# koadman/libMems

Hardware: AMD Instinct MI355X
Metric: seed-mers/sec sorted+matched (+ MUMs/sec) at 1/2/4/8 MI355X; HBM GB/s vs roofline (higher is better)
Workload: dtype u64; 1 GPU; BASELINE config 3: 8 x 100 Mbp, seed weight 19 (0x7b974ef), MemHash seed stage (sorted+matched); genomes=8, genome_length=100000000, seedmers_total=799999792, seedmers_rank0=799999792, probes_rank0=100459493, parallelism=1 GPU

## Files before the change

libmems_amd/csrc/groups.hip:

```cpp
#include <cstdlib>
#include <type_traits>

#include "match_device.h"
#include "seed_device.h"

namespace mums {

namespace {

constexpr int kGTile = kSegTile;
constexpr int kGRounds = kGTile / kBlock;
constexpr int kSlots = kGTile / 2;
#ifndef MUMS_GROUP_SPLIT
#define MUMS_GROUP_SPLIT 2
#endif
constexpr int kGSplit = MUMS_GROUP_SPLIT;
constexpr int kGSub = kGTile / kGSplit;
constexpr int kGSubRounds = kGSub / kBlock;
constexpr int kSubSlots = kGSub / 2;
static_assert(kGSub % kBlock == 0 && kGSubRounds * (kBlock / 64) <= 64, "probe sub-tile");

__device__ __forceinline__ uint32_t blk_excl_scan(uint32_t v, uint32_t* s_w, uint32_t* total) {
    const int lane = threadIdx.x & 63, wv = threadIdx.x >> 6;
    uint32_t inc = v;
    #pragma unroll
    for (int d = 1; d < 64; d <<= 1) {
        uint32_t t = __shfl_up(inc, d, 64);
        if (lane >= d) inc += t;
    }
    if (lane == 63) s_w[wv] = inc;
    __syncthreads();
    uint32_t pre = 0, tot = 0;
    #pragma unroll
    for (int w = 0; w < kBlock / 64; ++w) {
        const uint32_t x = s_w[w];
        pre += (w < wv) ? x : 0u;
        tot += x;
    }
    __syncthreads();
    *total = tot;
    return pre + inc - v;
}

template <int MG, typename View>
__global__ __launch_bounds__(kBlock) void probe_tile_kernel(View v, const SegTile* __restrict__ tiles, uint64_t N,
                                                            GenomeTable gt, MatchParams mp, int L,
                                                            uint32_t* __restrict__ tile_count,
                                                            uint64_t* __restrict__ slot_info,
                                                            uint32_t* __restrict__ slot_bucket,
                                                            DevCounters* __restrict__ ctr) {
    __shared__ uint16_t heads[kGTile];
    __shared__ uint32_t okb[kGTile];
    __shared__ uint16_t gsz16[kGTile];
    __shared__ uint32_t wcnt[kGRounds][kBlock / 64];
    __shared__ uint32_t s_w[kBlock / 64];
    __shared__ uint32_t s_red[2];
    const int lane = threadIdx.x & 63, wv = threadIdx.x >> 6;
    const SegTile td = tiles[blockIdx.x];
    if (td.count == 0) {
        if (threadIdx.x == 0) {
            tile_count[blockIdx.x] = 0;
            tile_count[gridDim.x + 32 + blockIdx.x] = 0;
        }
        return;
    }
    const uint64_t tile0 = td.start;
    const uint64_t lt = (lane == 0) ? 0ull : (~0ull >> (64 - lane));

    uint32_t hmask = 0;
    #pragma unroll
    for (int r = 0; r < kGRounds; ++r) {
        const uint32_t q = r * kBlock + threadIdx.x;
        const uint64_t i = tile0 + q;
        bool head = false;
        if (q < td.count) head = (i == td.bstart) || (v.gkey(i) != v.gkey(i - 1));
        hmask |= (head ? 1u : 0u) << r;
        const uint64_t bal = __ballot(head);
        if (lane == 0) wcnt[r][wv] = (uint32_t)__popcll(bal);
    }
    __syncthreads();
    if (threadIdx.x == 0) {
        uint32_t acc = 0;
        for (int r = 0; r < kGRounds; ++r)
            for (int w = 0; w < kBlock / 64; ++w) { const uint32_t c = wcnt[r][w]; wcnt[r][w] = acc; acc += c; }
        s_red[0] = acc;
    }
    __syncthreads();
    #pragma unroll
    for (int r = 0; r < kGRounds; ++r) {
        const bool head = (hmask >> r) & 1u;
        const uint64_t bal = __ballot(head);
        if (head) heads[wcnt[r][wv] + (uint32_t)__popcll(bal & lt)] = (uint16_t)(r * kBlock + threadIdx.x);
    }
    __syncthreads();
    const uint32_t H = s_red[0];

    uint32_t nrep = 0;
    const bool fast = mp.repeat_tol == 0 && mp.enum_tol == 1;
    for (uint32_t j = threadIdx.x; j < H; j += kBlock) {
        uint32_t gsz = 0;
        int64_t off = 0;
        bool ok;
        if (fast) {
            ok = probe_offset_fast<MG, View>(v, tile0 + heads[j], td.bend, gt, mp, L, &off, &gsz);
        } else {
            Mhe<MG> P;
            ok = build_probe<MG, View>(v, tile0 + heads[j], td.bend, gt, mp, L, P, &gsz);
            off = P.offset;
        }
        nrep += gsz > (uint32_t)kRepeatLimit;
        okb[j] = ok ? (0x80000000u | bucket_of(off, mp.table_size)) : 0u;
        gsz16[j] = (uint16_t)(gsz > 65535u ? 65535u : gsz);
    }
    if (nrep) atomicAdd(&ctr->repeat_limit, (unsigned long long)nrep);
    __syncthreads();

    uint32_t base = 0;
    const uint64_t sb = (uint64_t)blockIdx.x * kSlots;
    for (uint32_t c = 0; c < H; c += kBlock) {
        const uint32_t j = c + threadIdx.x;
        const uint32_t vv = j < H ? okb[j] : 0u;
        const uint32_t ok = vv >> 31;
        uint32_t tot;
        const uint32_t o = blk_excl_scan(ok, s_w, &tot);
        if (ok) {
            slot_info[sb + base + o] = (tile0 + heads[j]) | ((uint64_t)gsz16[j] << 32);
            slot_bucket[sb + base + o] = vv & 0x7FFFFFFFu;
        }
        base += tot;
    }
    if (threadIdx.x == 0) {
        tile_count[blockIdx.x] = base;
        tile_count[gridDim.x + 32 + blockIdx.x] = H;
    }
}

typedef __attribute__((address_space(3))) const uint64_t lds_u64;

template <int IB>
struct TileRecViewT {
    lds_u64* lds;
    const uint64_t* glob;
    uint64_t t0;
    uint32_t count;
    __device__ __forceinline__ uint64_t raw(uint64_t i) const {
        const uint64_t k = i - t0;
        return k < count ? lds[k] : glob[i];
    }
    __device__ __forceinline__ uint64_t gkey(uint64_t i) const { return raw(i) >> (IB + 1); }
    __device__ __forceinline__ uint32_t par(uint64_t i) const { return (uint32_t)(raw(i) >> IB) & 1u; }
    __device__ __forceinline__ uint64_t gidx(uint64_t i) const { return raw(i) & ((1ull << IB) - 1); }
    __device__ __forceinline__ RecFields get(uint64_t i) const {
        const uint64_t r = raw(i);
        return RecFields{r >> (IB + 1), (uint32_t)(r >> IB) & 1u, r & ((1ull << IB) - 1)};
    }
};

template <int MG, int IB, bool kGl = false, bool kFastOnly = false>
__global__ __launch_bounds__(kBlock) __attribute__((amdgpu_waves_per_eu(kGl ? 6 : 1))) void probe_tile_rec_kernel(const uint64_t* __restrict__ rec,
                                                                const SegTile* __restrict__ tiles, GenomeTable gt,
                                                                MatchParams mp, int L,
                                                                uint32_t* __restrict__ tile_count,
                                                                uint64_t* __restrict__ slot_info,
                                                                uint32_t* __restrict__ slot_bucket,
                                                                DevCounters* __restrict__ ctr,
                                                                double inv_table) {
    constexpr int kGRounds = kGSubRounds;
    __shared__ uint64_t srec[kGSub];
    __shared__ uint16_t heads[kSubSlots];
    __shared__ uint32_t wcnt[kGRounds * (kBlock / 64)];
    __shared__ uint32_t s_w[kBlock / 64];
    __shared__ uint32_t s_red[2];
    __shared__ uint64_t s_prev, s_next;
    __shared__ uint8_t s_gl[256];
    __shared__ uint32_t s_gb[kMaxG + 1];
    const int lane = threadIdx.x & 63, wv = threadIdx.x >> 6;
    const SegTile td = tiles[blockIdx.x / kGSplit];
    const uint32_t part0 = (blockIdx.x % kGSplit) * (uint32_t)kGSub;
    if (td.count <= part0) {
        if (threadIdx.x == 0) {
            tile_count[blockIdx.x] = 0;
            tile_count[gridDim.x + 32 + blockIdx.x] = 0;
        }
        return;
    }
    const uint64_t tile0 = td.start + part0;
    const uint32_t cnt = td.count - part0 < (uint32_t)kGSub ? td.count - part0 : (uint32_t)kGSub;
    const uint64_t lt = (lane == 0) ? 0ull : (~0ull >> (64 - lane));

    {
        uint64_t x[kGRounds];
        #pragma unroll
        for (int r = 0; r < kGRounds; ++r) {
            const uint32_t q = r * kBlock + threadIdx.x;
            x[r] = rec[tile0 + (q < cnt ? q : cnt - 1)];
        }
        #pragma unroll
        for (int r = 0; r < kGRounds; ++r) {
            const uint32_t q = r * kBlock + threadIdx.x;
            if (q < cnt) srec[q] = x[r];
        }
    }
    if (threadIdx.x == 0) s_prev = (tile0 > td.bstart) ? rec[tile0 - 1] : ~0ull;
    if (threadIdx.x == 64) s_next = (tile0 + cnt < td.bend) ? rec[tile0 + cnt] : ~0ull;
    constexpr bool use_gl = kGl && IB == 32;
    if constexpr (use_gl) {
        static_assert(kBlock >= 256 && kBlock > kMaxG, "one lookup entry per thread");
        if (threadIdx.x < gt.gl_n) s_gl[threadIdx.x] = gt.gl[threadIdx.x];
        if (threadIdx.x <= kMaxG) s_gb[threadIdx.x] = (uint32_t)gt.base[threadIdx.x];
    }
    const GLook glk{(lds_u8c*)s_gl, (lds_u32c*)s_gb, gt.gl_shift, gt.gl_n ? gt.gl_n - 1 : 0};
    __syncthreads();

    uint32_t hmask = 0, ngrp = 0;
    #pragma unroll
    for (int r = 0; r < kGRounds; ++r) {
        const uint32_t q = r * kBlock + threadIdx.x;
        bool keep = false;
        if (q < cnt) {
            const uint64_t here = srec[q] >> (IB + 1);
            const uint64_t prev = (q == 0) ? ((tile0 == td.bstart) ? ~0ull : (s_prev >> (IB + 1)))
                                           : (srec[q - 1] >> (IB + 1));
            const uint64_t next = (q + 1 < cnt) ? (srec[q + 1] >> (IB + 1)) : (s_next >> (IB + 1));
            const bool head = (q == 0 && tile0 == td.bstart) || here != prev;
            ngrp += head ? 1u : 0u;
            keep = head && next == here;
        }
        hmask |= (keep ? 1u : 0u) << r;
        const uint64_t bal = __ballot(keep);
        if (lane == 0) wcnt[r * (kBlock / 64) + wv] = (uint32_t)__popcll(bal);
    }
    __syncthreads();
    if (wv == 0) {
        constexpr int kE = kGRounds * (kBlock / 64);
        const uint32_t c0 = lane < kE ? wcnt[lane] : 0u;
        uint32_t inc = c0;
        #pragma unroll
        for (int d = 1; d < 64; d <<= 1) {
            const uint32_t t = __shfl_up(inc, d, 64);
            if (lane >= d) inc += t;
        }
        if (lane < kE) wcnt[lane] = inc - c0;
        if (lane == 63) s_red[0] = inc;
    }
    __syncthreads();
    #pragma unroll
    for (int r = 0; r < kGRounds; ++r) {
        const bool keep = (hmask >> r) & 1u;
        const uint64_t bal = __ballot(keep);
        if (keep) heads[wcnt[r * (kBlock / 64) + wv] + (uint32_t)__popcll(bal & lt)] = (uint16_t)(r * kBlock + threadIdx.x);
    }
    __syncthreads();
    const uint32_t H = s_red[0];

    const TileRecViewT<IB> v{(lds_u64*)srec, rec, tile0, cnt};
    const bool fast = kFastOnly || (mp.repeat_tol == 0 && mp.enum_tol == 1);
    const double inv_t = inv_table;
    const uint64_t sb = (uint64_t)blockIdx.x * kSubSlots;
    uint32_t nrep = 0, base = 0;
    for (uint32_t c = 0; c < H; c += kBlock) {
        const uint32_t j = c + threadIdx.x;
        bool ok = false;
        uint32_t gsz = 0, bkt = 0;
        uint64_t h = 0;
        if (j < H) {
            h = tile0 + heads[j];
            int64_t off = 0;
            if (fast) {
                const uint32_t q = heads[j];
                uint64_t xb[MG + 1];
                if (q + (uint32_t)gt.G < cnt) {
                    #pragma unroll
                    for (int k = 0; k <= MG; ++k) {
                        const uint32_t qk = q + ((uint32_t)k <= (uint32_t)gt.G ? (uint32_t)k : 0u);
                        xb[k] = ((uint32_t)k <= (uint32_t)gt.G) ? v.lds[qk] : ~0ull;
                    }
                } else {
                    #pragma unroll
                    for (int k = 0; k <= MG; ++k)
                        xb[k] = ((uint32_t)k <= (uint32_t)gt.G && h + k < td.bend) ? rec[h + k] : ~0ull;
                }
                ok = probe_fast_raw<MG, IB, use_gl>(xb, gt, mp, L, &off, &gsz, &glk);
                if (gsz > (uint32_t)gt.G) {
                    uint64_t i = h + gsz;
                    const uint32_t k0 = (uint32_t)(xb[0] >> (IB + 1));
                    while (i < td.bend && gsz <= (uint32_t)kRepeatLimit && (uint32_t)v.gkey(i) == k0) { ++gsz; ++i; }
                }
            } else if constexpr (!kFastOnly) {
                Mhe<MG> P;
                ok = build_probe<MG, TileRecViewT<IB>>(v, h, td.bend, gt, mp, L, P, &gsz);
                off = P.offset;
            }
            nrep += gsz > (uint32_t)kRepeatLimit;
            if (ok) bkt = bucket_of_fast(off, mp.table_size, inv_t);
        }
        uint32_t tot;
        const uint32_t o = blk_excl_scan(ok ? 1u : 0u, s_w, &tot);
        if (ok) {
            slot_info[sb + base + o] = h | ((uint64_t)(gsz > 65535u ? 65535u : gsz) << 32);
            slot_bucket[sb + base + o] = bkt;
        }
        base += tot;
    }
    if (nrep) atomicAdd(&ctr->repeat_limit, (unsigned long long)nrep);
    uint32_t gtot;
    (void)blk_excl_scan(ngrp, s_w, &gtot);
    if (threadIdx.x == 0) {
        tile_count[blockIdx.x] = base;
        tile_count[gridDim.x + 32 + blockIdx.x] = gtot;
    }
}

__global__ __launch_bounds__(kBlock) void probe_compact_kernel(const uint32_t* __restrict__ tile_count,
                                                               const uint32_t* __restrict__ tile_off,
                                                               const uint64_t* __restrict__ slot_info,
                                                               const uint32_t* __restrict__ slot_bucket,
                                                               uint64_t* __restrict__ probe_info,
                                                               uint32_t* __restrict__ probe_bucket,
                                                               uint32_t slots_per_block) {
    const uint32_t n = tile_count[blockIdx.x];
    const uint64_t o = tile_off[blockIdx.x];
    const uint64_t sb = (uint64_t)blockIdx.x * slots_per_block;
    for (uint32_t k = threadIdx.x; k < n; k += kBlock) {
        probe_info[o + k] = slot_info[sb + k];
        probe_bucket[o + k] = slot_bucket[sb + k];
    }
}

__global__ void flat_tiles_kernel(uint64_t N, uint64_t nt, SegTile* __restrict__ tiles) {
    const uint64_t t = (uint64_t)blockIdx.x * blockDim.x + threadIdx.x;
    if (t >= nt) return;
    SegTile d{};
    d.start = t * kGTile;
    d.bstart = 0;
    d.bend = N;
    const uint64_t rem = N - d.start;
    d.count = (uint32_t)(rem < (uint64_t)kGTile ? rem : (uint64_t)kGTile);
    d.hbase = 0;
    d.ntb = (uint32_t)nt;
    d.tb = (uint32_t)t;
    tiles[t] = d;
}

#ifndef MUMS_MAT_WIDE
#define MUMS_MAT_WIDE 1
#endif
constexpr bool kMatWide = MUMS_MAT_WIDE != 0;
struct __attribute__((aligned(8))) Rec2 { uint64_t a, b; };

template <int MG, typename View, bool kGl = false>
__global__ __launch_bounds__(kBlock) void probe_materialize_kernel(View v, const uint64_t* __restrict__ probe_info,
                                                                   uint64_t P, GenomeTable gt, MatchParams mp, int L,
                                                                   int64_t* __restrict__ rows, uint64_t* __restrict__ lkey,
                                                                   uint32_t* __restrict__ fsk, uint32_t* __restrict__ lhash,
                                                                   int32_t* __restrict__ rows32) {
    const uint64_t k0 = (uint64_t)blockIdx.x * kBlock;
    const uint64_t k = k0 + threadIdx.x;
    const int W = gt.G + 1;
    Mhe<MG> Q;
    __shared__ uint8_t s_gl[256];
    __shared__ uint32_t s_gb[kMaxG + 1];
    constexpr bool use_gl = kGl && RecIB<View>::value == 32;
    if constexpr (use_gl) {
        for (uint32_t i = threadIdx.x; i < gt.gl_n; i += kBlock) s_gl[i] = gt.gl[i];
        for (int i = threadIdx.x; i <= kMaxG; i += kBlock) s_gb[i] = (uint32_t)gt.base[i];
        __syncthreads();
    }
    const GLook glk{(lds_u8c*)s_gl, (lds_u32c*)s_gb, gt.gl_shift, gt.gl_n ? gt.gl_n - 1 : 0};
    if (k < P) {
        const uint64_t info = probe_info[k];
        const uint64_t h = info & 0xFFFFFFFFull;
        const uint32_t gsz = (uint32_t)((info >> 32) & 0xFFFFull);
        bool done = false;
        if constexpr (RecIB<View>::value > 0) {
            if (mp.repeat_tol == 0 && mp.enum_tol == 1 && gsz <= (uint32_t)MG) {
                uint64_t x[MG];
                if constexpr (MG % 2 == 0 && kMatWide) {
                    #pragma unroll
                    for (int q = 0; q < MG; q += 2) {
                        Rec2 t{~0ull, ~0ull};
                        if ((uint32_t)q < gsz) t = *reinterpret_cast<const Rec2*>(v.rec + h + q);
                        x[q] = t.a;
                        x[q + 1] = (uint32_t)(q + 1) < gsz ? t.b : ~0ull;
                    }
                } else {
                    #pragma unroll
                    for (int q = 0; q < MG; ++q) x[q] = (uint32_t)q < gsz ? v.rec[h + q] : ~0ull;
                }
                probe_row_fast<MG, RecIB<View>::value, use_gl>(x, gsz, gt, L, Q, &glk);
                done = true;
            }
        }
        if (!done) {
            uint32_t gs;
            build_probe<MG, View>(v, h, h + gsz, gt, mp, L, Q, &gs);
        }
        if (lkey) {
            const uint64_t xs = (uint64_t)start_at(Q, first_start(Q));
            if (lhash) {
                lkey[k] = (xs << 32) | k;
                lhash[k] = line_hash<MG>(Q, gt.G);
            } else {
                lkey[k] = ((uint64_t)line_hash<MG>(Q, gt.G) << 32) | (xs & 0xFFFFFFFFull);
            }
            fsk[k] = (uint32_t)xs;
        }
    }
    if constexpr (MG % 4 == 0 && MG <= 16) {
        if (rows32) {
            if (k >= P) return;
            bool ok = probe_offset<MG>(Q, L) == Q.offset;
            #pragma unroll
            for (int g = 0; g < MG; ++g) ok = ok && Q.s[g] == (int64_t)(int32_t)Q.s[g];
            int32_t* out = rows32 + k * (uint64_t)line_row_stride(gt.G);
            #pragma unroll
            for (int q = 0; q < MG / 4; ++q)
                if (4 * q < gt.G)
                    *reinterpret_cast<int4*>(out + 4 * q) = make_int4((int32_t)Q.s[4 * q], (int32_t)Q.s[4 * q + 1],
                                                                      (int32_t)Q.s[4 * q + 2], (int32_t)Q.s[4 * q + 3]);
            if (!ok) atomicOr(fsk + P, 1u);
            return;
        }
    }
    if constexpr (MG <= 16) {
        __shared__ int64_t srow[kBlock * (MG + 1)];
        if (k < P) {
            int64_t* r = srow + threadIdx.x * W;
            #pragma unroll
            for (int g = 0; g < MG; ++g)
                if (g < gt.G) r[g] = Q.s[g];
            r[gt.G] = Q.offset;
        }
        __syncthreads();
        const uint64_t nk = P - k0 < (uint64_t)kBlock ? P - k0 : (uint64_t)kBlock;
        int64_t* out = rows + k0 * (uint64_t)W;
        for (uint32_t i = threadIdx.x; i < nk * (uint64_t)W; i += kBlock) out[i] = srow[i];
    } else {
        if (k >= P) return;
        int64_t* row = rows + k * (uint64_t)W;
        #pragma unroll
        for (int g = 0; g < MG; ++g)
            if (g < gt.G) row[g] = Q.s[g];
        row[gt.G] = Q.offset;
    }
}

__global__ __launch_bounds__(kBlock) void row_bucket_kernel(const int64_t* __restrict__ rows, uint64_t P, int G,
                                                            uint32_t table_size, double inv_t,
                                                            const uint32_t* __restrict__ bounds, uint32_t nranks,
                                                            uint32_t* __restrict__ out) {
    const uint64_t k = (uint64_t)blockIdx.x * kBlock + threadIdx.x;
    if (k >= P) return;
    const uint32_t b = bucket_of_fast(rows[k * (uint64_t)(G + 1) + G], table_size, inv_t);
    if (!bounds) { out[k] = b; return; }
    uint32_t r = 0;
    while (r + 1 < nranks && bounds[r + 1] <= b) ++r;
    out[k] = r;
}

constexpr int kGatherIPT = 8;
__global__ __launch_bounds__(kBlock) void gather_rows_ilp_kernel(const int64_t* __restrict__ src,
                                                                 const uint32_t* __restrict__ perm, uint64_t n, uint32_t W,
                                                                 int64_t* __restrict__ dst) {
    const uint64_t e0 = (uint64_t)blockIdx.x * (kBlock * kGatherIPT) + threadIdx.x;
    uint64_t k = e0 / W;
    uint32_t c = (uint32_t)(e0 - k * W);
    const uint32_t dk = kBlock / W, dc = kBlock % W;
    int64_t x[kGatherIPT];
    #pragma unroll
    for (int i = 0; i < kGatherIPT; ++i) {
        const uint64_t e = e0 + (uint64_t)i * kBlock;
        x[i] = e < n ? src[(uint64_t)perm[k] * W + c] : 0;
        k += dk;
        c += dc;
        if (c >= W) { c -= W; ++k; }
    }
    #pragma unroll
    for (int i = 0; i < kGatherIPT; ++i) {
        const uint64_t e = e0 + (uint64_t)i * kBlock;
        if (e < n) dst[e] = x[i];
    }
}

__global__ __launch_bounds__(kBlock) void bucket_rec_kernel(const uint32_t* __restrict__ b, uint64_t P,
                                                            uint64_t* __restrict__ rec) {
    const uint64_t k = (uint64_t)blockIdx.x * kBlock + threadIdx.x;
    if (k < P) rec[k] = ((uint64_t)b[k] << 32) | k;
}

__global__ __launch_bounds__(kBlock) void bucket_split_kernel(const uint64_t* __restrict__ rec, uint64_t P,
                                                              uint32_t* __restrict__ b, uint32_t* __restrict__ ids) {
    const uint64_t k = (uint64_t)blockIdx.x * kBlock + threadIdx.x;
    if (k >= P) return;
    const uint64_t r = rec[k];
    b[k] = (uint32_t)(r >> 32);
    ids[k] = (uint32_t)r;
}

__global__ __launch_bounds__(kBlock) void chain_dest_kernel(const uint32_t* __restrict__ fk, uint64_t nch,
                                                            const uint32_t* __restrict__ pdest,
                                                            uint32_t* __restrict__ cdest) {
    const uint64_t c = (uint64_t)blockIdx.x * kBlock + threadIdx.x;
    if (c < nch) cdest[c] = pdest[fk[c]];
}

__global__ __launch_bounds__(kBlock) void inverse_perm_kernel(const uint32_t* __restrict__ perm, uint64_t n,
                                                              uint32_t* __restrict__ inv) {
    const uint64_t k = (uint64_t)blockIdx.x * kBlock + threadIdx.x;
    if (k < n) inv[perm[k]] = (uint32_t)k;
}

__global__ __launch_bounds__(kBlock) void chain_tag_kernel(const uint32_t* __restrict__ chain_of,
                                                           const uint32_t* __restrict__ perm,
                                                           const uint32_t* __restrict__ sdest, uint64_t P,
                                                           const uint32_t* __restrict__ cinv,
                                                           const uint32_t* __restrict__ cstart,
                                                           uint32_t* __restrict__ tags) {
    const uint64_t k = (uint64_t)blockIdx.x * kBlock + threadIdx.x;
    if (k < P) tags[k] = cinv[chain_of[perm[k]]] - cstart[sdest[k]];
}

__global__ __launch_bounds__(kBlock) void chain_entry_out_kernel(const int64_t* __restrict__ pool,
                                                                 const uint32_t* __restrict__ fk,
                                                                 const uint32_t* __restrict__ cperm,
                                                                 const uint32_t* __restrict__ scdest, uint64_t nch,
                                                                 int G, const uint32_t* __restrict__ pinv,
                                                                 const uint32_t* __restrict__ rstart,
                                                                 int64_t* __restrict__ eout, uint32_t* __restrict__ fout) {
    const uint64_t k = (uint64_t)blockIdx.x * kBlock + threadIdx.x;
    if (k >= nch) return;
    const uint32_t c = cperm[k];
    const uint64_t W = (uint64_t)(G + 2);
    for (uint64_t w = 0; w < W; ++w) eout[k * W + w] = pool[(uint64_t)c * W + w];
    if (fout) fout[k] = pinv[fk[c]] - rstart[scdest[k]];
}

__global__ __launch_bounds__(kBlock) void kept_dest_kernel(const int64_t* __restrict__ rows, uint64_t P, int G,
                                                           const uint32_t* __restrict__ chain_of,
                                                           const uint32_t* __restrict__ cinv,
                                                           const uint2* __restrict__ thr,
                                                           const uint32_t* __restrict__ fk,
                                                           const uint32_t* __restrict__ pdest, uint32_t nranks,
                                                           uint32_t* __restrict__ dest) {
    const uint64_t k = (uint64_t)blockIdx.x * kBlock + threadIdx.x;
    if (k >= P) return;
    const uint32_t c = chain_of[k];
    const uint2 t = thr[cinv[c]];
    bool keep = t.y != 0u && fk[c] == (uint32_t)k;
    if (!keep) {
        const int64_t* r = rows + k * (uint64_t)(G + 1);
        int64_t fs = 0;
        for (int g = 0; g < G && fs == 0; ++g) fs = r[g];
        keep = (uint64_t)fs >= (uint64_t)t.x;
    }
    dest[k] = keep ? pdest[k] : nranks + pdest[k];
}

__global__ __launch_bounds__(kBlock) void dest_first_kernel(const uint32_t* __restrict__ sdest, uint64_t P,
                                                            uint32_t* __restrict__ first) {
    const uint64_t i = (uint64_t)blockIdx.x * kBlock + threadIdx.x;
    if (i < P && (i == 0 || sdest[i - 1] != sdest[i])) first[sdest[i]] = (uint32_t)i;
}

__global__ __launch_bounds__(kBlock) void entry_first_init_kernel(const uint32_t* __restrict__ scdest, uint64_t nch,
                                                                  const uint32_t* __restrict__ rcount,
                                                                  uint32_t* __restrict__ efirst) {
    const uint64_t x = (uint64_t)blockIdx.x * kBlock + threadIdx.x;
    if (x < nch) efirst[x] = rcount[scdest[x]];
}

__global__ __launch_bounds__(kBlock) void entry_first_kernel(const uint32_t* __restrict__ perm,
                                                             const uint32_t* __restrict__ sdest, uint64_t K,
                                                             const uint32_t* __restrict__ chain_of,
                                                             const uint32_t* __restrict__ cinv,
                                                             const uint32_t* __restrict__ rstart,
                                                             uint32_t* __restrict__ efirst) {
    const uint64_t i = (uint64_t)blockIdx.x * kBlock + threadIdx.x;
    if (i < K) atomicMin(&efirst[cinv[chain_of[perm[i]]]], (uint32_t)i - rstart[sdest[i]]);
}

template <typename I, int IB>
__global__ __launch_bounds__(kBlock) void rec_pairs_kernel(const uint64_t* __restrict__ rec, uint64_t n,
                                                           const uint32_t* __restrict__ bst, uint32_t nb,
                                                           uint32_t kfirst, int kb_rec, uint64_t* __restrict__ key,
                                                           I* __restrict__ idx) {
    const uint64_t i = (uint64_t)blockIdx.x * kBlock + threadIdx.x;
    if (i >= n) return;
    uint32_t lo = 0, hi = nb;
    while (lo < hi) {
        const uint32_t mid = (lo + hi + 1) >> 1;
        if (bst[mid] <= i) lo = mid;
        else hi = mid - 1;
    }
    const uint64_t r = rec[i];
    key[i] = ((uint64_t)(kfirst + lo) << kb_rec) | (r >> IB);
    idx[i] = (I)(r & ((1ull << IB) - 1));
}

}

hipError_t launch_rec_pairs(const uint64_t* rec, uint64_t n, const uint32_t* d_bst, uint32_t nb, uint32_t kfirst,
                            int kb_rec, uint64_t* key, uint32_t* idx, hipStream_t st) {
    if (n == 0) return hipSuccess;
    hipLaunchKernelGGL((rec_pairs_kernel<uint32_t, 32>), dim3((unsigned)((n + kBlock - 1) / kBlock)), dim3(kBlock), 0, st,
                       rec, n, d_bst, nb, kfirst, kb_rec, key, idx);
    return hipGetLastError();
}

hipError_t launch_rec_pairs33(const uint64_t* rec, uint64_t n, const uint32_t* d_bst, uint32_t nb, uint32_t kfirst,
                              int kb_rec, uint64_t* key, uint64_t* idx, hipStream_t st) {
// ... 206 lines not shown
```

libmems_amd/csrc/match_device.h:

```cpp
#pragma once

#include <type_traits>

#include "mums_internal.h"
#include "seed_device.h"

namespace mums {

template <int MG>
struct Mhe {
    int64_t len;
    int64_t offset;
    int64_t mersize;
    int64_t s[MG];
};

template <int MG>
__device__ __forceinline__ int first_start(const Mhe<MG>& m) {
    int f = MG;
    #pragma unroll
    for (int g = MG - 1; g >= 0; --g) f = (m.s[g] != 0) ? g : f;
    return f;
}

template <int MG>
__device__ __forceinline__ int64_t start_at(const Mhe<MG>& m, int i) {
    int64_t v = 0;
    #pragma unroll
    for (int g = 0; g < MG; ++g) v = (g == i) ? m.s[g] : v;
    return v;
}

template <int MG>
__device__ __forceinline__ bool mhe_contains(const Mhe<MG>& a, const Mhe<MG>& b) {
    if (a.offset != b.offset) return false;
    const int i = first_start(b);
    const int64_t ai = start_at(a, i), bi = start_at(b, i);
    if (ai == 0) return false;
    const int64_t diff = bi - ai;
    if (diff < 0 || (uint64_t)a.len < (uint64_t)(b.len + diff)) return false;
    const int64_t diff_rc = b.len - a.len + diff;
    bool ok = true;
    #pragma unroll
    for (int g = 0; g < MG; ++g) {
        if (g <= i) continue;
        const int64_t di = b.s[g] - a.s[g];
        if (b.s[g] == 0 && a.s[g] == 0) continue;
        if (b.s[g] < 0 && diff_rc == di) continue;
        if (diff != di) ok = false;
    }
    return ok;
}

template <int MG>
__device__ __forceinline__ bool mhe_strict_lt(const Mhe<MG>& a, const Mhe<MG>& b) {
    const int start_diff = first_start(a) - first_start(b);
    if (start_diff == 0) {
        int res = -1;
        #pragma unroll
        for (int g = 0; g < MG; ++g) {
            int64_t as = a.s[g], bs = b.s[g];
            if (as < 0) as = -as + a.len - a.mersize;
            if (bs < 0) bs = -bs + b.len - b.mersize;
            const int64_t d = as - bs;
            if (res < 0 && d != 0) res = d < 0 ? 1 : 0;
        }
        if (res >= 0) return res == 1;
    }
    return start_diff < 0;
}

template <int MG>
__device__ __forceinline__ bool mhe_less(const Mhe<MG>& a, const Mhe<MG>& b) {
    const int fa = first_start(a), fb = first_start(b);
    if (fa > fb) return true;
    if (fa != fb) return false;
    int res = -1;
    #pragma unroll
    for (int g = 0; g < MG; ++g) {
        const bool az = a.s[g] == 0, bz = b.s[g] == 0;
        if (res < 0 && az && !bz) res = 1;
        if (res < 0 && !az && bz) res = 0;
    }
    if (res >= 0) return res == 1;
    if (mhe_contains(a, b) || mhe_contains(b, a)) return false;
    return mhe_strict_lt(a, b);
}

template <int MG>
__device__ __forceinline__ void load_entry(const int64_t* __restrict__ pool, uint32_t id, int G, Mhe<MG>& e) {
    const int64_t* p = pool + (uint64_t)id * (uint64_t)(G + 2);
    e.len = p[0];
    e.offset = p[1];
    e.mersize = 0;
    #pragma unroll
    for (int g = 0; g < MG; ++g) e.s[g] = (g < G) ? p[2 + g] : 0;
}

template <int MG>
__device__ __forceinline__ uint32_t lower_bound_tbl(const uint32_t* tbl, uint32_t t, const int64_t* __restrict__ pool,
                                                   int G, const Mhe<MG>& val) {
    uint32_t first = 0, len = t;
    Mhe<MG> e;
    while (len > 0) {
        const uint32_t half = len >> 1, mid = first + half;
        load_entry(pool, tbl[mid], G, e);
        if (mhe_less(e, val)) {
            first = mid + 1;
            len = len - half - 1;
        } else {
            len = half;
        }
    }
    return first;
}

template <int MG, typename View>
__device__ __forceinline__ bool build_probe(const View& v, uint64_t h, uint64_t end, const GenomeTable& gt,
                                            const MatchParams& mp, int L, Mhe<MG>& P, uint32_t* gsize) {
    const uint64_t k0 = v.gkey(h);
    const uint32_t maxc = (uint32_t)gt.G * (mp.repeat_tol + 1u);
    uint32_t tally[MG];
    int64_t pos1[MG];
    uint32_t par[MG];
    #pragma unroll
    for (int g = 0; g < MG; ++g) { tally[g] = 0; pos1[g] = 0; par[g] = 0; }
    uint32_t cnt = 0, nh = 0;
    bool reject = false;
    for (uint64_t i = h; i < end; ++i) {
        if (v.gkey(i) != k0) break;
        ++cnt;
        if (cnt > maxc) {
            reject = true;
            if (cnt > (uint32_t)kRepeatLimit) break;
            continue;
        }
        if (reject) continue;
        const uint64_t gi = v.gidx(i);
        const int g = genome_of(gt, gi);
        const int64_t p = (int64_t)(gi - gt.base[g]);
        const uint32_t pb = v.par(i);
        #pragma unroll
        for (int q = 0; q < MG; ++q) {
            if (q != g) continue;
            if (tally[q] < mp.enum_tol) { pos1[q] = p + 1; par[q] = pb; ++nh; }
            if (tally[q] > mp.repeat_tol) reject = true;
            ++tally[q];
        }
    }
    *gsize = cnt;
    if (reject || cnt < 2 || nh < 2) return false;
    P.len = L;
    P.mersize = L;
    #pragma unroll
    for (int g = 0; g < MG; ++g) P.s[g] = pos1[g];
    const int ref = first_start(P);
    uint32_t ref_par = 0;
    #pragma unroll
    for (int g = 0; g < MG; ++g) ref_par = (g == ref) ? par[g] : ref_par;
    #pragma unroll
    for (int g = 0; g < MG; ++g)
        if (g > ref && P.s[g] != 0 && par[g] != ref_par) P.s[g] = -P.s[g];
    const int64_t sref = start_at(P, ref);
    int64_t off = 0;
    uint64_t match_number = 0;
    int mult = 0;
    #pragma unroll
    for (int g = 0; g < MG; ++g) {
        if (g > ref && P.s[g] != 0) off += P.s[g] - sref - (P.s[g] < 0 ? (int64_t)L : 0);
        if (g < gt.G) {
            match_number = (match_number << 1) | (P.s[g] != 0 ? 1ull : 0ull);
            mult += P.s[g] != 0;
        }
    }
    P.offset = off;
    if (mp.masked) return mp.seq_mask == 0 || match_number == mp.seq_mask;
    return mult >= 2;
}

template <int MG>
__device__ __forceinline__ int genome_of_mg(const GenomeTable& gt, uint64_t i) {
    int g = 0;
    #pragma unroll
    for (int k = 1; k < MG; ++k) g += (k < gt.G && i >= gt.base[k]) ? 1 : 0;
    return g;
}

template <int MG>
using MaskT = typename std::conditional<(MG > 32), uint64_t, uint32_t>::type;

template <typename M>
__device__ __forceinline__ uint64_t match_number_of(M mask, uint32_t G) {
    if constexpr (sizeof(M) == 8) return __builtin_bitreverse64(mask) >> (64 - G);
    else return (uint64_t)(__builtin_bitreverse32(mask) >> (32 - G));
}

template <int MG, typename View>
__device__ __forceinline__ bool probe_offset_batch(const RecFields (&r)[MG + 1], const View& v, uint64_t h,
                                                   uint64_t end, const GenomeTable& gt, const MatchParams& mp, int L,
                                                   int64_t* offset, uint32_t* gsize) {
    const uint32_t G = (uint32_t)gt.G;
    const uint64_t k0 = r[0].gk;
    uint32_t cnt = 0;
    bool run = true;
    #pragma unroll
    for (int k = 0; k <= MG; ++k) {
        run = run && (r[k].gk == k0);
        cnt += run ? 1u : 0u;
    }
    if (cnt > G) {
        uint64_t i = h + cnt;
        while (i < end && cnt <= (uint32_t)kRepeatLimit && v.gkey(i) == k0) { ++cnt; ++i; }
        *gsize = cnt;
        return false;
    }
    *gsize = cnt;
    if (cnt < 2) return false;
    MaskT<MG> mask = 0;
    bool dup = false;
    int gref = 64;
    int64_t sref = 0;
    uint32_t pref = 0;
    int gk[MG + 1];
    #pragma unroll
    for (int k = 0; k <= MG; ++k) {
        gk[k] = genome_of_mg<MG>(gt, r[k].idx);
        if ((uint32_t)k < cnt) {
            const int g = gk[k];
            dup = dup || ((mask >> g) & 1u);
            mask |= (MaskT<MG>)1 << g;
            if (g < gref) {
                gref = g;
                sref = (int64_t)(r[k].idx - gt.base[g]) + 1;
                pref = r[k].par;
            }
        }
    }
    if (dup) return false;
    int64_t off = 0;
    #pragma unroll
    for (int k = 0; k <= MG; ++k) {
        if ((uint32_t)k < cnt && gk[k] != gref) {
            const int64_t s = (int64_t)(r[k].idx - gt.base[gk[k]]) + 1;
            off += (r[k].par != pref) ? (-s - sref - (int64_t)L) : (s - sref);
        }
    }
    *offset = off;
    if (mp.masked) {
        const uint64_t match_number = match_number_of(mask, G);
        return mp.seq_mask == 0 || match_number == mp.seq_mask;
    }
    return true;
}

template <int MG, typename View>
__device__ __forceinline__ bool probe_offset_fast(const View& v, uint64_t h, uint64_t end, const GenomeTable& gt,
                                                  const MatchParams& mp, int L, int64_t* offset, uint32_t* gsize) {
    RecFields r[MG + 1];
    #pragma unroll
    for (int k = 0; k <= MG; ++k)
        r[k] = ((uint32_t)k <= (uint32_t)gt.G && h + k < end) ? v.get(h + k) : RecFields{~0ull, 0u, 0u};
    return probe_offset_batch<MG, View>(r, v, h, end, gt, mp, L, offset, gsize);
}

__device__ __forceinline__ uint32_t bucket_of_fast(int64_t offset, uint32_t table_size, double inv_t) {
    const int64_t T = (int64_t)table_size;
    const int64_t q = (int64_t)floor((double)offset * inv_t);
    int64_t r = offset - q * T;
    r = r < 0 ? r + T : r;
    r = r >= T ? r - T : r;
    return (uint32_t)r;
}

typedef __attribute__((address_space(3))) const uint8_t lds_u8c;
typedef __attribute__((address_space(3))) const uint32_t lds_u32c;
struct GLook {
    lds_u8c* tab;
    lds_u32c* base;
    uint32_t shift, last;
};
__device__ __forceinline__ void glook(const GLook& l, uint32_t idx, uint32_t* g, uint32_t* b) {
    const uint32_t s = min(idx >> l.shift, l.last);
    const uint32_t t = l.tab[s];
    const uint32_t b0 = l.base[t], b1 = l.base[t + 1];
    const bool ge = idx >= b1;
    *g = t + (ge ? 1u : 0u);
    *b = ge ? b1 : b0;
}

template <int MG, int IB = 32, bool kGl = false>
__device__ __forceinline__ bool probe_fast_raw(const uint64_t (&x)[MG + 1], const GenomeTable& gt,
                                               const MatchParams& mp, int L, int64_t* offset, uint32_t* gsize,
                                               const GLook* glk = nullptr) {
    const uint32_t G = (uint32_t)gt.G;
    const uint32_t k0 = (uint32_t)(x[0] >> (IB + 1));
    uint32_t cnt = 0;
    bool run = true;
    #pragma unroll
    for (int k = 0; k <= MG; ++k) {
        run = run && ((uint32_t)(x[k] >> (IB + 1)) == k0) && (x[k] != ~0ull);
        cnt += run ? 1u : 0u;
    }
    *gsize = cnt;
    MaskT<MG> mask = 0;
    uint32_t gref = 64, pref = 0;
    using IdxT = typename std::conditional<(IB > 32), uint64_t, uint32_t>::type;
    IdxT sref = 0;
    bool dup = false;
    uint32_t gk[MG];
    IdxT sk[MG];
    #pragma unroll
    for (int k = 0; k < MG; ++k) {
        const IdxT idx = (IdxT)(x[k] & ((1ull << IB) - 1));
        uint32_t g = 0;
        IdxT b = 0;
        if constexpr (kGl && IB == 32) {
            uint32_t bb;
            glook(*glk, (uint32_t)idx, &g, &bb);
            b = bb;
        } else {
            #pragma unroll
            for (int j = 1; j < MG; ++j) {
                const IdxT bj = (IdxT)gt.base[j];
                const bool ge = (uint32_t)j < G && idx >= bj;
                g = ge ? (uint32_t)j : g;
                b = ge ? bj : b;
            }
        }
        gk[k] = g;
        sk[k] = idx - b + 1u;
        const bool in = (uint32_t)k < cnt;
        dup = dup || (in && ((mask >> g) & 1u));
        mask |= in ? ((MaskT<MG>)1 << g) : (MaskT<MG>)0;
        const bool better = in && g < gref;
        gref = better ? g : gref;
        sref = better ? sk[k] : sref;
        pref = better ? (uint32_t)(x[k] >> IB) & 1u : pref;
    }
    int64_t off = 0;
    #pragma unroll
    for (int k = 0; k < MG; ++k) {
        const bool use = (uint32_t)k < cnt && gk[k] != gref;
        const int64_t sv = (int64_t)sk[k], sr = (int64_t)sref;
        const int64_t term = (((uint32_t)(x[k] >> IB) & 1u) != pref) ? (-sv - sr - (int64_t)L) : (sv - sr);
        off += use ? term : 0;
    }
    *offset = off;
    const bool accept = cnt >= 2 && cnt <= G && !dup;
    if (mp.masked) {
        const uint64_t match_number = match_number_of(mask, G);
        return accept && (mp.seq_mask == 0 || match_number == mp.seq_mask);
    }
    return accept;
}

template <int MG, int IB = 32, bool kGl = false>
__device__ __forceinline__ void probe_row_fast(const uint64_t (&x)[MG], uint32_t cnt, const GenomeTable& gt, int L,
                                               Mhe<MG>& P, const GLook* glk = nullptr) {
    using IdxT = typename std::conditional<(IB > 32), uint64_t, uint32_t>::type;
    const uint32_t G = (uint32_t)gt.G;
    int64_t st[MG];
    uint32_t gk[MG], pk[MG];
    #pragma unroll
    for (int k = 0; k < MG; ++k) {
        const IdxT idx = (IdxT)(x[k] & ((1ull << IB) - 1));
        uint32_t g = 0;
        IdxT b = 0;
        if constexpr (kGl && IB == 32) {
            uint32_t bb;
            glook(*glk, (uint32_t)idx, &g, &bb);
            b = bb;
        } else {
            #pragma unroll
            for (int j = 1; j < MG; ++j) {
                const IdxT bj = (IdxT)gt.base[j];
                const bool ge = (uint32_t)j < G && idx >= bj;
                g = ge ? (uint32_t)j : g;
                b = ge ? bj : b;
            }
        }
        gk[k] = (uint32_t)k < cnt ? g : 0xFFu;
        pk[k] = (uint32_t)(x[k] >> IB) & 1u;
        st[k] = (int64_t)(idx - b) + 1;
    }
    uint32_t gref = 0xFFu, ref_par = 0;
    int64_t sref = 0;
    #pragma unroll
    for (int k = 0; k < MG; ++k) {
        const bool better = gk[k] < gref;
        gref = better ? gk[k] : gref;
        ref_par = better ? pk[k] : ref_par;
        sref = better ? st[k] : sref;
    }
    int64_t off = 0;
    #pragma unroll
    for (int k = 0; k < MG; ++k) {
        const bool other = gk[k] != gref && gk[k] != 0xFFu;
        const bool rev = other && pk[k] != ref_par;
        st[k] = rev ? -st[k] : st[k];
        off += other ? (st[k] - sref - (rev ? (int64_t)L : 0)) : 0;
    }
    P.len = L;
    P.mersize = L;
    P.offset = off;
    #pragma unroll
    for (int g = 0; g < MG; ++g) {
        int64_t v = 0;
        #pragma unroll
        for (int k = 0; k < MG; ++k) v = gk[k] == (uint32_t)g ? st[k] : v;
        P.s[g] = v;
    }
}

__device__ __forceinline__ uint64_t mix64(uint64_t x) {
    x ^= x >> 30;
    x *= 0xbf58476d1ce4e5b9ull;
    x ^= x >> 27;
    x *= 0x94d049bb133111ebull;
    x ^= x >> 31;
    return x;
}

#ifndef MUMS_LINE_HASH_BITS
#define MUMS_LINE_HASH_BITS 32
#endif
constexpr int kLineHashBits = MUMS_LINE_HASH_BITS;
template <int MG>
__device__ __forceinline__ uint64_t line_hash64(const Mhe<MG>& P, int G) {
    const int ref = first_start(P);
    const int64_t x = start_at(P, ref);
    uint64_t h = 0x9e3779b97f4a7c15ull ^ (uint64_t)ref;
    #pragma unroll
    for (int g = 0; g < MG; ++g) {
        if (g < G && g > ref && P.s[g] != 0) {
            const int64_t s = P.s[g];
            const uint64_t d = s > 0 ? (uint64_t)(s - x) : (uint64_t)(-s + x) ^ 0x8000000000000000ull;
            h = mix64(h ^ d ^ ((uint64_t)g << 56));
        } else {
            h = mix64(h ^ ((uint64_t)g << 48));
        }
    }
    return h;
}
template <int MG>
__device__ __forceinline__ uint32_t line_hash(const Mhe<MG>& P, int G) {
    return (uint32_t)(line_hash64<MG>(P, G) >> (64 - kLineHashBits));
}


struct MatProbes {
    const int64_t* rows;
    const uint32_t* fs = nullptr;
    const int32_t* rows32 = nullptr;
    uint32_t stride32 = 0;
    int L32 = 0;
};

template <int MG>
__device__ __forceinline__ int64_t probe_offset(const Mhe<MG>& P, int L) {
    const int ref = first_start(P);
    const int64_t sref = start_at(P, ref);
    int64_t off = 0;
    #pragma unroll
    for (int g = 0; g < MG; ++g)
        if (g > ref && P.s[g] != 0) off += P.s[g] - sref - (P.s[g] < 0 ? (int64_t)L : 0);
    return off;
}

__host__ __device__ inline uint32_t line_row_stride(int G) { return (uint32_t)((G + 3) & ~3); }

template <int MG>
__device__ __forceinline__ void load_probe32(const int32_t* __restrict__ row, int G, int L, int Loff, Mhe<MG>& P) {
    P.len = L;
    P.mersize = L;
    if constexpr (MG % 4 == 0) {
        #pragma unroll
        for (int q = 0; q < MG / 4; ++q) {
            int4 v = make_int4(0, 0, 0, 0);
            if (4 * q < G) v = *reinterpret_cast<const int4*>(row + 4 * q);
            P.s[4 * q] = v.x;
            P.s[4 * q + 1] = 4 * q + 1 < G ? v.y : 0;
            P.s[4 * q + 2] = 4 * q + 2 < G ? v.z : 0;
            P.s[4 * q + 3] = 4 * q + 3 < G ? v.w : 0;
        }
    } else {
        #pragma unroll
        for (int g = 0; g < MG; ++g) P.s[g] = (g < G) ? row[g] : 0;
    }
    P.offset = probe_offset<MG>(P, Loff);
}

template <int MG>
__device__ __forceinline__ void load_probe(const MatProbes& m, uint64_t k, int G, int L, Mhe<MG>& P) {
    if (m.rows32) {
        load_probe32<MG>(m.rows32 + k * (uint64_t)m.stride32, G, L, m.L32, P);
        return;
    }
    const int64_t* row = m.rows + k * (uint64_t)(G + 1);
    P.len = L;
    P.mersize = L;
    P.offset = row[G];
    #pragma unroll
    for (int g = 0; g < MG; ++g) P.s[g] = (g < G) ? row[g] : 0;
}

struct LineRows {
    const int32_t* rows;
    uint32_t stride;
    int L;
    const uint32_t* ord = nullptr;
};

template <int MG>
__device__ __forceinline__ void load_probe(const LineRows& m, uint64_t k, int G, int L, Mhe<MG>& P) {
    const uint64_t r = m.ord ? (uint64_t)m.ord[k] : k;
    load_probe32<MG>(m.rows + r * (uint64_t)m.stride, G, L, m.L, P);
}

__device__ __forceinline__ uint32_t bucket_of(int64_t offset, uint32_t table_size) {
    const int64_t T = (int64_t)table_size;
    return (uint32_t)(((offset % T) + T) % T);
}

}
```

Before: 37.87 billion seed-mers/s.

## Streamline probe kernel with DPP neighbors, mbcnt ranks, and closed-form offset

Result: faster. 38.55 billion seed-mers/s (median of 6 runs) (+1.8%).

```diff
diff --git a/libmems_amd/csrc/groups.hip b/libmems_amd/csrc/groups.hip
--- a/libmems_amd/csrc/groups.hip
+++ b/libmems_amd/csrc/groups.hip
@@ -166,15 +166,18 @@
                                                                 DevCounters* __restrict__ ctr,
                                                                 double inv_table) {
     constexpr int kGRounds = kGSubRounds;
+    constexpr int kWaves = kBlock / 64;
     __shared__ uint64_t srec[kGSub];
     __shared__ uint16_t heads[kSubSlots];
-    __shared__ uint32_t wcnt[kGRounds * (kBlock / 64)];
-    __shared__ uint32_t s_w[kBlock / 64];
+    __shared__ uint32_t wcnt[kGRounds * kWaves];
+    __shared__ uint32_t s_w[2][kWaves];
+    __shared__ uint32_t s_ng[kWaves];
     __shared__ uint32_t s_red[2];
     __shared__ uint64_t s_prev, s_next;
     __shared__ uint8_t s_gl[256];
     __shared__ uint32_t s_gb[kMaxG + 1];
-    const int lane = threadIdx.x & 63, wv = threadIdx.x >> 6;
+    const int lane = threadIdx.x & 63;
+    const int wv = __builtin_amdgcn_readfirstlane(threadIdx.x >> 6);
     const SegTile td = tiles[blockIdx.x / kGSplit];
     const uint32_t part0 = (blockIdx.x % kGSplit) * (uint32_t)kGSub;
     if (td.count <= part0) {
@@ -186,8 +189,8 @@
     }
     const uint64_t tile0 = td.start + part0;
     const uint32_t cnt = td.count - part0 < (uint32_t)kGSub ? td.count - part0 : (uint32_t)kGSub;
-    const uint64_t lt = (lane == 0) ? 0ull : (~0ull >> (64 - lane));
-
+
+    uint32_t kx[kGRounds];
     {
         uint64_t x[kGRounds];
         #pragma unroll
@@ -199,6 +202,7 @@
         for (int r = 0; r < kGRounds; ++r) {
             const uint32_t q = r * kBlock + threadIdx.x;
             if (q < cnt) srec[q] = x[r];
+            kx[r] = (uint32_t)(x[r] >> (IB + 1));
         }
     }
     if (threadIdx.x == 0) s_prev = (tile0 > td.bstart) ? rec[tile0 - 1] : ~0ull;
@@ -212,27 +216,38 @@
     const GLook glk{(lds_u8c*)s_gl, (lds_u32c*)s_gb, gt.gl_shift, gt.gl_n ? gt.gl_n - 1 : 0};
     __syncthreads();
 
+    const bool first = tile0 == td.bstart;
+    const uint32_t kprev = (uint32_t)(s_prev >> (IB + 1)), knext = (uint32_t)(s_next >> (IB + 1));
+    uint32_t ke[kGRounds];
+    #pragma unroll
+    for (int r = 0; r < kGRounds; ++r) ke[r] = 0;
+    if (lane == 0 || lane == 63) {
+        #pragma unroll
+        for (int r = 0; r < kGRounds; ++r) {
+            const uint32_t q = r * kBlock + threadIdx.x;
+            const uint32_t qe = lane == 0 ? q - 1 : q + 1;
+            ke[r] = qe < cnt ? (uint32_t)(srec[qe] >> (IB + 1)) : (lane == 0 ? kprev : knext);
+        }
+    }
     uint32_t hmask = 0, ngrp = 0;
     #pragma unroll
     for (int r = 0; r < kGRounds; ++r) {
         const uint32_t q = r * kBlock + threadIdx.x;
-        bool keep = false;
-        if (q < cnt) {
-            const uint64_t here = srec[q] >> (IB + 1);
-            const uint64_t prev = (q == 0) ? ((tile0 == td.bstart) ? ~0ull : (s_prev >> (IB + 1)))
-                                           : (srec[q - 1] >> (IB + 1));
-            const uint64_t next = (q + 1 < cnt) ? (srec[q + 1] >> (IB + 1)) : (s_next >> (IB + 1));
-            const bool head = (q == 0 && tile0 == td.bstart) || here != prev;
-            ngrp += head ? 1u : 0u;
-            keep = head && next == here;
-        }
+        const uint32_t here = kx[r];
+        const uint32_t prev = (uint32_t)__builtin_amdgcn_update_dpp((int)ke[r], (int)here, 0x138, 0xf, 0xf, false);
+        uint32_t next = (uint32_t)__builtin_amdgcn_update_dpp((int)ke[r], (int)here, 0x130, 0xf, 0xf, false);
+        next = (q + 1 < cnt) ? next : knext;
+        const bool head = q < cnt && ((q == 0 && first) || here != prev);
+        const bool keep = head && next == here;
+        ngrp += (uint32_t)__popcll(__ballot(head));
         hmask |= (keep ? 1u : 0u) << r;
         const uint64_t bal = __ballot(keep);
-        if (lane == 0) wcnt[r * (kBlock / 64) + wv] = (uint32_t)__popcll(bal);
-    }
+        if (lane == 0) wcnt[r * kWaves + wv] = (uint32_t)__popcll(bal);
+    }
+    if (lane == 0) s_ng[wv] = ngrp;
     __syncthreads();
     if (wv == 0) {
-        constexpr int kE = kGRounds * (kBlock / 64);
+        constexpr int kE = kGRounds * kWaves;
         const uint32_t c0 = lane < kE ? wcnt[lane] : 0u;
         uint32_t inc = c0;
         #pragma unroll
@@ -248,16 +263,18 @@
     for (int r = 0; r < kGRounds; ++r) {
         const bool keep = (hmask >> r) & 1u;
         const uint64_t bal = __ballot(keep);
-        if (keep) heads[wcnt[r * (kBlock / 64) + wv] + (uint32_t)__popcll(bal & lt)] = (uint16_t)(r * kBlock + threadIdx.x);
+        const uint32_t below = __builtin_amdgcn_mbcnt_hi((uint32_t)(bal >> 32), __builtin_amdgcn_mbcnt_lo((uint32_t)bal, 0u));
+        if (keep) heads[wcnt[r * kWaves + wv] + below] = (uint16_t)(r * kBlock + threadIdx.x);
     }
     __syncthreads();
     const uint32_t H = s_red[0];
 
     const TileRecViewT<IB> v{(lds_u64*)srec, rec, tile0, cnt};
     const bool fast = kFastOnly || (mp.repeat_tol == 0 && mp.enum_tol == 1);
+    const uint64_t want_mn = mp.masked ? mp.seq_mask : 0ull;
     const double inv_t = inv_table;
     const uint64_t sb = (uint64_t)blockIdx.x * kSubSlots;
-    uint32_t nrep = 0, base = 0;
+    uint32_t nrep = 0, base = 0, buf = 0;
     for (uint32_t c = 0; c < H; c += kBlock) {
         const uint32_t j = c + threadIdx.x;
         bool ok = false;
@@ -280,7 +297,7 @@
                     for (int k = 0; k <= MG; ++k)
                         xb[k] = ((uint32_t)k <= (uint32_t)gt.G && h + k < td.bend) ? rec[h + k] : ~0ull;
                 }
-                ok = probe_fast_raw<MG, IB, use_gl>(xb, gt, mp, L, &off, &gsz, &glk);
+                ok = probe_fast_raw<MG, IB, use_gl>(xb, gt, want_mn, L, &off, &gsz, &glk);
                 if (gsz > (uint32_t)gt.G) {
                     uint64_t i = h + gsz;
                     const uint32_t k0 = (uint32_t)(xb[0] >> (IB + 1));
@@ -294,18 +311,30 @@
             nrep += gsz > (uint32_t)kRepeatLimit;
             if (ok) bkt = bucket_of_fast(off, mp.table_size, inv_t);
         }
-        uint32_t tot;
-        const uint32_t o = blk_excl_scan(ok ? 1u : 0u, s_w, &tot);
+        const uint64_t bal = __ballot(ok);
+        const uint32_t below = __builtin_amdgcn_mbcnt_hi((uint32_t)(bal >> 32), __builtin_amdgcn_mbcnt_lo((uint32_t)bal, 0u));
+        if (lane == 0) s_w[buf][wv] = (uint32_t)__popcll(bal);
+        __syncthreads();
+        uint32_t pre = 0, tot = 0;
+        #pragma unroll
+        for (int w = 0; w < kWaves; ++w) {
+            const uint32_t x = s_w[buf][w];
+            pre += (w < wv) ? x : 0u;
+            tot += x;
+        }
+        buf ^= 1u;
         if (ok) {
-            slot_info[sb + base + o] = h | ((uint64_t)(gsz > 65535u ? 65535u : gsz) << 32);
-            slot_bucket[sb + base + o] = bkt;
+            const uint32_t o = base + pre + below;
+            slot_info[sb + o] = h | ((uint64_t)(gsz > 65535u ? 65535u : gsz) << 32);
+            slot_bucket[sb + o] = bkt;
         }
         base += tot;
     }
     if (nrep) atomicAdd(&ctr->repeat_limit, (unsigned long long)nrep);
-    uint32_t gtot;
-    (void)blk_excl_scan(ngrp, s_w, &gtot);
     if (threadIdx.x == 0) {
+        uint32_t gtot = 0;
+        #pragma unroll
+        for (int w = 0; w < kWaves; ++w) gtot += s_ng[w];
         tile_count[blockIdx.x] = base;
         tile_count[gridDim.x + 32 + blockIdx.x] = gtot;
     }
diff --git a/libmems_amd/csrc/match_device.h b/libmems_amd/csrc/match_device.h
--- a/libmems_amd/csrc/match_device.h
+++ b/libmems_amd/csrc/match_device.h
@@ -288,9 +288,33 @@
     *b = ge ? b1 : b0;
 }
 
+template <int MG, int IB, bool kGl, typename IdxT>
+__device__ __forceinline__ void rec_genome_start(uint64_t x, const GenomeTable& gt, const GLook* glk, uint32_t* g_out,
+                                                 IdxT* s_out) {
+    const IdxT idx = (IdxT)(x & ((1ull << IB) - 1));
+    uint32_t g = 0;
+    IdxT b = 0;
+    if constexpr (kGl && IB == 32) {
+        uint32_t bb;
+        glook(*glk, (uint32_t)idx, &g, &bb);
+        b = bb;
+    } else {
+        const uint32_t G = (uint32_t)gt.G;
+        #pragma unroll
+        for (int j = 1; j < MG; ++j) {
+            const IdxT bj = (IdxT)gt.base[j];
+            const bool ge = (uint32_t)j < G && idx >= bj;
+            g = ge ? (uint32_t)j : g;
+            b = ge ? bj : b;
+        }
+    }
+    *g_out = g;
+    *s_out = idx - b + 1u;
+}
+
 template <int MG, int IB = 32, bool kGl = false>
-__device__ __forceinline__ bool probe_fast_raw(const uint64_t (&x)[MG + 1], const GenomeTable& gt,
-                                               const MatchParams& mp, int L, int64_t* offset, uint32_t* gsize,
+__device__ __forceinline__ bool probe_fast_raw(const uint64_t (&x)[MG + 1], const GenomeTable& gt, uint64_t want_mn,
+                                               int L, int64_t* offset, uint32_t* gsize,
                                                const GLook* glk = nullptr) {
     const uint32_t G = (uint32_t)gt.G;
     const uint32_t k0 = (uint32_t)(x[0] >> (IB + 1));
@@ -303,54 +327,36 @@
     }
     *gsize = cnt;
     MaskT<MG> mask = 0;
-    uint32_t gref = 64, pref = 0;
+    uint32_t gref = 64, pref = 0, n1 = 0;
     using IdxT = typename std::conditional<(IB > 32), uint64_t, uint32_t>::type;
     IdxT sref = 0;
-    bool dup = false;
-    uint32_t gk[MG];
-    IdxT sk[MG];
+    uint64_t tot = 0, sum1 = 0;
     #pragma unroll
     for (int k = 0; k < MG; ++k) {
-        const IdxT idx = (IdxT)(x[k] & ((1ull << IB) - 1));
-        uint32_t g = 0;
-        IdxT b = 0;
-        if constexpr (kGl && IB == 32) {
-            uint32_t bb;
-            glook(*glk, (uint32_t)idx, &g, &bb);
-            b = bb;
-        } else {
-            #pragma unroll
-            for (int j = 1; j < MG; ++j) {
-                const IdxT bj = (IdxT)gt.base[j];
-                const bool ge = (uint32_t)j < G && idx >= bj;
-                g = ge ? (uint32_t)j : g;
-                b = ge ? bj : b;
-            }
-        }
-        gk[k] = g;
-        sk[k] = idx - b + 1u;
+        uint32_t g;
+        IdxT s;
+        rec_genome_start<MG, IB, kGl, IdxT>(x[k], gt, glk, &g, &s);
         const bool in = (uint32_t)k < cnt;
-        dup = dup || (in && ((mask >> g) & 1u));
+        const uint32_t par = (uint32_t)(x[k] >> IB) & 1u;
+        const IdxT d = in ? s : (IdxT)0;
+        const uint32_t pin = in ? par : 0u;
         mask |= in ? ((MaskT<MG>)1 << g) : (MaskT<MG>)0;
         const bool better = in && g < gref;
         gref = better ? g : gref;
-        sref = better ? sk[k] : sref;
-        pref = better ? (uint32_t)(x[k] >> IB) & 1u : pref;
-    }
-    int64_t off = 0;
-    #pragma unroll
-    for (int k = 0; k < MG; ++k) {
-        const bool use = (uint32_t)k < cnt && gk[k] != gref;
-        const int64_t sv = (int64_t)sk[k], sr = (int64_t)sref;
-        const int64_t term = (((uint32_t)(x[k] >> IB) & 1u) != pref) ? (-sv - sr - (int64_t)L) : (sv - sr);
-        off += use ? term : 0;
-    }
-    *offset = off;
-    const bool accept = cnt >= 2 && cnt <= G && !dup;
-    if (mp.masked) {
-        const uint64_t match_number = match_number_of(mask, G);
-        return accept && (mp.seq_mask == 0 || match_number == mp.seq_mask);
-    }
+        sref = better ? s : sref;
+        pref = better ? par : pref;
+        tot += d;
+        sum1 += pin ? d : (IdxT)0;
+        n1 += pin;
+    }
+    const uint64_t dif = tot - 2 * sum1;
+    const uint32_t nrev = pref ? cnt - n1 : n1;
+    *offset = (int64_t)((pref ? 0 - dif : dif) - (uint64_t)cnt * (uint64_t)sref - (uint64_t)(nrev * (uint32_t)L));
+    uint32_t npres;
+    if constexpr (sizeof(MaskT<MG>) == 8) npres = (uint32_t)__popcll(mask);
+    else npres = (uint32_t)__popc(mask);
+    bool accept = cnt >= 2 && cnt <= G && npres == cnt;
+    if (want_mn) accept = accept && match_number_of(mask, G) == want_mn;
     return accept;
 }
 
@@ -358,30 +364,16 @@
 __device__ __forceinline__ void probe_row_fast(const uint64_t (&x)[MG], uint32_t cnt, const GenomeTable& gt, int L,
                                                Mhe<MG>& P, const GLook* glk = nullptr) {
     using IdxT = typename std::conditional<(IB > 32), uint64_t, uint32_t>::type;
-    const uint32_t G = (uint32_t)gt.G;
     int64_t st[MG];
     uint32_t gk[MG], pk[MG];
     #pragma unroll
     for (int k = 0; k < MG; ++k) {
-        const IdxT idx = (IdxT)(x[k] & ((1ull << IB) - 1));
-        uint32_t g = 0;
-        IdxT b = 0;
-        if constexpr (kGl && IB == 32) {
-            uint32_t bb;
-            glook(*glk, (uint32_t)idx, &g, &bb);
-            b = bb;
-        } else {
-            #pragma unroll
-            for (int j = 1; j < MG; ++j) {
-                const IdxT bj = (IdxT)gt.base[j];
-                const bool ge = (uint32_t)j < G && idx >= bj;
-                g = ge ? (uint32_t)j : g;
-                b = ge ? bj : b;
-            }
-        }
+        uint32_t g;
+        IdxT s;
+        rec_genome_start<MG, IB, kGl, IdxT>(x[k], gt, glk, &g, &s);
         gk[k] = (uint32_t)k < cnt ? g : 0xFFu;
         pk[k] = (uint32_t)(x[k] >> IB) & 1u;
-        st[k] = (int64_t)(idx - b) + 1;
+        st[k] = (int64_t)s;
     }
     uint32_t gref = 0xFFu, ref_par = 0;
     int64_t sref = 0;
```
